# facebookresearch/atlas

Hardware: NVIDIA B200
Metric: end-to-end queries/sec (retrieve top-40 + FiD-base fwd) (higher is better)
Workload: dtype bf16

## Files before the change

### atlas_b200/csrc/gemm.cu

```cuda
#include "common.cuh"
#include "host_common.h"

#include <math.h>
#include <stdlib.h>

namespace gemm {

constexpr int BLOCK_M = 128;
constexpr int BLOCK_K = 64;
constexpr int UMMA_K = 16;
constexpr int THREADS = 384;
constexpr int EPI_WARPS = 8;

enum Epilogue { EPI_NONE = 0, EPI_BIAS = 1, EPI_GELU = 2, EPI_RESIDUAL = 3, EPI_GATED = 4 };

template <int BLOCK_N, bool kPair>
struct Cfg {
    static constexpr int CTAS = kPair ? 2 : 1;
    static constexpr int A_BYTES = BLOCK_M * BLOCK_K * 2;
    static constexpr int B_ROWS = BLOCK_N / CTAS;
    static constexpr int B_BYTES = B_ROWS * BLOCK_K * 2;
    static constexpr int STAGE_BYTES = A_BYTES + B_BYTES;
    static constexpr int STAGES = (192 * 1024) / STAGE_BYTES;
    static constexpr int EPI_STAGE_BYTES = BLOCK_N == 256 ? EPI_WARPS * 4096 : 0;
    static constexpr int SMEM_BYTES = STAGES * STAGE_BYTES + EPI_STAGE_BYTES + 1024;
    static constexpr int TMEM_COLS = 2 * BLOCK_N;
    static constexpr int UMMA_M = BLOCK_M * CTAS;
};

struct Params {
    int M, N, K;
    int ldc;
    int ldr;
    int epi;
    const uint16_t* bias;
    const uint16_t* residual;
    uint16_t* C;
    const float* row_ss;
    float* out_ss;
    float rs_eps;
    int splits, kb_per_split;
    float* C32;
    int l2_prefetch;
    int tma_store;
    const int32_t* m_dev;
};

template <bool kBF16>
__device__ __forceinline__ float to_f32(uint16_t h) {
    if constexpr (kBF16) return __bfloat162float(__ushort_as_bfloat16(h));
    return __half2float(__ushort_as_half(h));
}
template <bool kBF16>
__device__ __forceinline__ uint32_t pack2(float a, float b) {
    return ab::pack2_rn<kBF16>(a, b);
}

__device__ __forceinline__ float gelu_erf(float x) {
    const float z = fabsf(x) * 0.70710678118654752f;
    float t, e;
    asm("rcp.approx.ftz.f32 %0, %1;" : "=f"(t) : "f"(fmaf(0.3275911f, z, 1.0f)));
    asm("ex2.approx.ftz.f32 %0, %1;" : "=f"(e) : "f"(-1.4426950408889634f * z * z));
    float poly = fmaf(1.061405429f, t, -1.453152027f);
    poly = fmaf(poly, t, 1.421413741f);
    poly = fmaf(poly, t, -0.284496736f);
    poly = fmaf(poly, t, 0.254829592f);
    const float erfc_abs = poly * t * e;
    const float one_plus_erf = x >= 0.f ? 2.0f - erfc_abs : erfc_abs;
    return 0.5f * x * one_plus_erf;
}
__device__ __forceinline__ float gelu_new(float x) {
    const float u2 = x * (1.5957691216057308f + 0.07135481627260025f * x * x);
    float e, r;
    asm("ex2.approx.ftz.f32 %0, %1;" : "=f"(e) : "f"(-1.4426950408889634f * u2));
    asm("rcp.approx.ftz.f32 %0, %1;" : "=f"(r) : "f"(1.0f + e));
    return x * r;
}

__device__ __forceinline__ uint64_t umma_desc_mn_sw128(uint32_t smem_addr, uint32_t lbo_bytes) {
    uint64_t d = 0;
    d |= static_cast<uint64_t>((smem_addr & 0x3FFFFu) >> 4);
    d |= static_cast<uint64_t>(lbo_bytes >> 4) << 16;
    d |= static_cast<uint64_t>(1024 >> 4) << 32;
    d |= static_cast<uint64_t>(1) << 46;
    d |= static_cast<uint64_t>(2) << 61;
    return d;
}

template <bool kBF16, int BLOCK_N, bool kPair, bool kTN, bool kQuad>
__global__ void __launch_bounds__(THREADS, 1)
gemm_kernel(const __grid_constant__ CUtensorMap tmap_a, const __grid_constant__ CUtensorMap tmap_b,
            const __grid_constant__ CUtensorMap tmap_c, const Params p) {
    using C = Cfg<BLOCK_N, kPair>;
    extern __shared__ uint8_t smem_raw[];
    __shared__ __align__(8) uint64_t full_bar[C::STAGES];
    __shared__ __align__(8) uint64_t empty_bar[C::STAGES];
    __shared__ __align__(8) uint64_t tmem_full_bar[2];
    __shared__ __align__(8) uint64_t tmem_empty_bar[2];
    __shared__ uint32_t tmem_base_smem;

    const uint32_t warp = threadIdx.x >> 5;
    const uint32_t lane = threadIdx.x & 31u;
    const uint32_t smem_base = (ab::smem_u32(smem_raw) + 1023u) & ~1023u;
    uint8_t* smem_gen = smem_raw + (smem_base - ab::smem_u32(smem_raw));

    static_assert(!kQuad || (kPair && !kTN), "the 4-CTA cluster builds on the K-major pair kernel");
    constexpr int CLUSTER = kQuad ? 4 : (kPair ? 2 : 1);
    const uint32_t cluster_rank = kPair ? ab::cluster_ctarank() : 0u;
    const uint32_t cta_rank = cluster_rank & 1u;
    const uint32_t pair_id = kQuad ? (cluster_rank >> 1) : 0u;
    const bool leader = cta_rank == 0;
    const int group = static_cast<int>(blockIdx.x) / CLUSTER;
    const int num_groups = static_cast<int>(gridDim.x) / CLUSTER;
    constexpr int PAIR_M = BLOCK_M * C::CTAS;
    constexpr int TILE_M = PAIR_M * (kQuad ? 2 : 1);
    const int m_rows = p.m_dev != nullptr ? min(p.M, max(__ldg(p.m_dev), 0)) : p.M;
    const int num_m = (m_rows + TILE_M - 1) / TILE_M;
    const int num_n = (p.N + BLOCK_N - 1) / BLOCK_N;
    const int num_tiles = num_m * num_n * p.splits;
    const int num_kb = (p.K + BLOCK_K - 1) / BLOCK_K;

    if (warp == 0 && lane == 0) {
        ab::tma_prefetch_desc(&tmap_a);
        ab::tma_prefetch_desc(&tmap_b);
    }
    if (warp == 1 && lane == 0) {
        for (int s = 0; s < C::STAGES; ++s) {
            ab::mbar_init(&full_bar[s], 1);
            ab::mbar_init(&empty_bar[s], kQuad ? 2 : 1);
        }
        for (int b = 0; b < 2; ++b) {
            ab::mbar_init(&tmem_full_bar[b], 1);
            ab::mbar_init(&tmem_empty_bar[b], EPI_WARPS * C::CTAS);
        }
        ab::fence_barrier_init();
    }
    if (warp == 2) ab::tmem_alloc<C::CTAS>(&tmem_base_smem, C::TMEM_COLS);
    ab::tc_fence_before();
    if constexpr (kPair) {
        ab::cluster_sync_all();
    } else {
        __syncthreads();
    }
    ab::tc_fence_after();
    const uint32_t tmem_base = tmem_base_smem;

    if (warp == 0) {
        if (lane == 0) {
            uint32_t stage = 0, phase = 0;
            for (int t = group; t < num_tiles; t += num_groups) {
                const int tile = t / p.splits, split = t % p.splits;
                const int m_blk = tile / num_n, n_blk = tile % num_n;
                const int a_row = m_blk * TILE_M + static_cast<int>(pair_id) * PAIR_M + static_cast<int>(cta_rank) * BLOCK_M;
                const int b_row = n_blk * BLOCK_N + static_cast<int>(cta_rank) * C::B_ROWS;
                const int kb0 = split * p.kb_per_split, kb1 = min(num_kb, kb0 + p.kb_per_split);
                int pf_row = -1;
                if constexpr (!kTN) {
                    const int t2 = t + num_groups;
                    if (p.l2_prefetch && t2 < num_tiles && (t2 / p.splits) % num_n == 0)
                        pf_row = ((t2 / p.splits) / num_n) * TILE_M + static_cast<int>(pair_id) * PAIR_M +
                                 static_cast<int>(cta_rank) * BLOCK_M;
                }
                for (int kb = kb0; kb < kb1; ++kb) {
                    if (pf_row >= 0) ab::tma_prefetch_2d(&tmap_a, kb * BLOCK_K, pf_row);
                    ab::mbar_wait(&empty_bar[stage], phase ^ 1u, 11);
                    uint8_t* st = smem_gen + stage * C::STAGE_BYTES;
                    if constexpr (kTN) {
                        if constexpr (kPair) {
                            if (leader) ab::mbar_arrive_expect_tx(&full_bar[stage], 2 * C::STAGE_BYTES);
                        } else {
                            ab::mbar_arrive_expect_tx(&full_bar[stage], C::STAGE_BYTES);
                        }
#pragma unroll
                        for (int j = 0; j < BLOCK_M / 64; ++j) {
                            if constexpr (kPair)
                                ab::tma_load_2d_2sm(&tmap_a, &full_bar[stage], st + j * 8192, a_row + 64 * j, kb * BLOCK_K,
                                                    ab::kEvictNormal);
                            else
                                ab::tma_load_2d(&tmap_a, &full_bar[stage], st + j * 8192, a_row + 64 * j, kb * BLOCK_K,
                                                ab::kEvictNormal);
                        }
#pragma unroll
                        for (int j = 0; j < C::B_ROWS / 64; ++j) {
                            if constexpr (kPair)
                                ab::tma_load_2d_2sm(&tmap_b, &full_bar[stage], st + C::A_BYTES + j * 8192, b_row + 64 * j,
                                                    kb * BLOCK_K, ab::kEvictNormal);
                            else
                                ab::tma_load_2d(&tmap_b, &full_bar[stage], st + C::A_BYTES + j * 8192, b_row + 64 * j,
                                                kb * BLOCK_K, ab::kEvictNormal);
                        }
                    } else if constexpr (kQuad) {
                        if (leader) ab::mbar_arrive_expect_tx(&full_bar[stage], 2 * C::STAGE_BYTES);
                        ab::tma_load_2d_2sm(&tmap_a, &full_bar[stage], st, kb * BLOCK_K, a_row, ab::kEvictNormal);
                        ab::tma_load_2d_2sm_mc(&tmap_b, &full_bar[stage], st + C::A_BYTES + pair_id * (64 * BLOCK_K * 2),
                                               kb * BLOCK_K, b_row + static_cast<int>(pair_id) * 64,
                                               static_cast<uint16_t>(0x5u << cta_rank), ab::kEvictLast);
                    } else if constexpr (kPair) {
                        if (leader) ab::mbar_arrive_expect_tx(&full_bar[stage], 2 * C::STAGE_BYTES);
                        ab::tma_load_2d_2sm(&tmap_a, &full_bar[stage], st, kb * BLOCK_K, a_row, ab::kEvictNormal);
                        ab::tma_load_2d_2sm(&tmap_b, &full_bar[stage], st + C::A_BYTES, kb * BLOCK_K, b_row,
                                            ab::kEvictLast);
                    } else {
                        ab::mbar_arrive_expect_tx(&full_bar[stage], C::STAGE_BYTES);
                        ab::tma_load_2d(&tmap_a, &full_bar[stage], st, kb * BLOCK_K, a_row, ab::kEvictNormal);
                        ab::tma_load_2d(&tmap_b, &full_bar[stage], st + C::A_BYTES, kb * BLOCK_K, b_row,
                                        ab::kEvictLast);
                    }
                    if (++stage == C::STAGES) {
                        stage = 0;
                        phase ^= 1u;
                    }
                }
            }
        }
    } else if (warp == 1) {
        if (lane == 0 && leader) {
            constexpr uint32_t idesc = ab::umma_idesc_f16(C::UMMA_M, BLOCK_N, kBF16) | (kTN ? ((1u << 15) | (1u << 16)) : 0u);
            uint32_t stage = 0, phase = 0;
            int it = 0;
            for (int t = group; t < num_tiles; t += num_groups, ++it) {
                const uint32_t buf = it & 1;
                ab::mbar_wait(&tmem_empty_bar[buf], ((it >> 1) & 1) ^ 1u, 12);
                ab::tc_fence_after();
                const uint32_t d_tmem = tmem_base + buf * BLOCK_N;
                const int kb0 = (t % p.splits) * p.kb_per_split, kb1 = min(num_kb, kb0 + p.kb_per_split);
                for (int kb = kb0; kb < kb1; ++kb) {
                    ab::mbar_wait(&full_bar[stage], phase, 13);
                    ab::tc_fence_after();
                    if constexpr (kTN) {
                        const uint64_t adesc0 = umma_desc_mn_sw128(smem_base + stage * C::STAGE_BYTES, 8192);
                        const uint64_t bdesc0 = umma_desc_mn_sw128(smem_base + stage * C::STAGE_BYTES + C::A_BYTES, 8192);
#pragma unroll
                        for (int k = 0; k < BLOCK_K / UMMA_K; ++k) {
                            ab::umma_ss<C::CTAS>(d_tmem, adesc0 + ((k * UMMA_K * 128) >> 4),
                                                 bdesc0 + ((k * UMMA_K * 128) >> 4), idesc, ((kb - kb0) | k) != 0 ? 1u : 0u);
                        }
                    } else {
                        const uint64_t adesc0 = ab::umma_desc_k_sw128(smem_base + stage * C::STAGE_BYTES);
                        const uint64_t bdesc0 = ab::umma_desc_k_sw128(smem_base + stage * C::STAGE_BYTES + C::A_BYTES);
#pragma unroll
                        for (int k = 0; k < BLOCK_K / UMMA_K; ++k) {
                            ab::umma_ss<C::CTAS>(d_tmem, adesc0 + ((k * UMMA_K * 2) >> 4),
                                                 bdesc0 + ((k * UMMA_K * 2) >> 4), idesc, ((kb - kb0) | k) != 0 ? 1u : 0u);
                        }
                    }
                    if constexpr (kQuad) {
                        ab::umma_commit_2sm(&empty_bar[stage], 0xF);
                    } else if constexpr (kPair) {
                        ab::umma_commit_2sm(&empty_bar[stage], 0x3);
                    } else {
                        ab::umma_commit(&empty_bar[stage]);
                    }
                    if (++stage == C::STAGES) {
                        stage = 0;
                        phase ^= 1u;
                    }
                }
                if constexpr (kPair) {
                    ab::umma_commit_2sm(&tmem_full_bar[buf], static_cast<uint16_t>(0x3u << (2 * pair_id)));
                } else {
                    ab::umma_commit(&tmem_full_bar[buf]);
                }
            }
        }
    } else if (warp >= 4) {
        const uint32_t lg = warp & 3u;
        const uint32_t half = (warp - 4u) >> 2;
        constexpr int CHUNKS = BLOCK_N / 64;
        int it = 0;
        for (int t = group; t < num_tiles; t += num_groups, ++it) {
            const uint32_t buf = it & 1;
            const int tile = t / p.splits, split = t % p.splits;
            const int m_blk = tile / num_n, n_blk = tile % num_n;
            const int row = m_blk * TILE_M + static_cast<int>(pair_id) * PAIR_M + static_cast<int>(cta_rank) * BLOCK_M +
                            static_cast<int>(lg * 32 + lane);
            const float rscale = (p.row_ss != nullptr && row < p.M)
                                     ? rsqrtf(__ldg(p.row_ss + row) / static_cast<float>(p.K) + p.rs_eps) : 1.0f;
            float ss_out = 0.f;
            if constexpr (BLOCK_N == 256) {
                if (p.tma_store && p.C32 == nullptr) {
                    uint8_t* stg = smem_gen + C::STAGES * C::STAGE_BYTES + (warp - 4u) * 4096u;
                    const uint32_t swz = lane & 7u;
                    const bool gated = p.epi == EPI_GATED;
                    const int n_groups = gated ? 1 : 2;
                    const int row_warp = m_blk * TILE_M + static_cast<int>(pair_id) * PAIR_M + static_cast<int>(cta_rank) * BLOCK_M +
                                         static_cast<int>(lg * 32);
                    const int acc_col_w = static_cast<int>(half) * (BLOCK_N / 2);
                    const int out_col_w = gated ? n_blk * (BLOCK_N / 2) + static_cast<int>(half) * (BLOCK_N / 4)
                                                : n_blk * BLOCK_N + acc_col_w;
                    const bool use_res = p.epi == EPI_RESIDUAL;
                    uint4 rq[8];
                    auto load_res = [&](int g) {
#pragma unroll
                        for (int i = 0; i < 8; ++i) {
                            const int rr = row_warp + static_cast<int>(lane >> 3) + 4 * i;
                            const int cc = out_col_w + g * 64 + static_cast<int>(lane & 7u) * 8;
                            rq[i] = (rr < p.M && cc < p.N)
                                        ? __ldg(reinterpret_cast<const uint4*>(p.residual + static_cast<size_t>(rr) * p.ldr + cc))
                                        : make_uint4(0u, 0u, 0u, 0u);
                        }
                    };
                    if (use_res) load_res(0);
                    ab::mbar_wait(&tmem_full_bar[buf], (it >> 1) & 1, 14);
                    ab::tc_fence_after();
#pragma unroll 1
                    for (int g = 0; g < n_groups; ++g) {
                        if (lane == 0) ab::tma_store_wait_read();
                        __syncwarp();
                        uint4 rown[8];
                        if (use_res) {
#pragma unroll
                            for (int i = 0; i < 8; ++i) {
                                const uint32_t rr = (lane >> 3) + 4u * i;
                                *reinterpret_cast<uint4*>(stg + rr * 128u + (((lane & 7u) ^ (rr & 7u)) << 4)) = rq[i];
                            }
                            __syncwarp();
#pragma unroll
                            for (int k = 0; k < 8; ++k)
                                rown[k] = *reinterpret_cast<const uint4*>(stg + lane * 128u + ((static_cast<uint32_t>(k) ^ swz) << 4));
                            if (g + 1 < n_groups) load_res(g + 1);
                        }
                        const int chunks_in_group = gated ? 4 : 2;
#pragma unroll 1
                        for (int cg = 0; cg < chunks_in_group; ++cg) {
                            const int c = gated ? cg : g * 2 + cg;
                            const int col_local = acc_col_w + c * 32;
                            const int col0 = n_blk * BLOCK_N + col_local;
                            uint32_t r[32];
                            ab::tmem_ld32(tmem_base + ((lg * 32u) << 16) + buf * BLOCK_N + col_local, r);
                            ab::tmem_ld_wait();
                            if (c == CHUNKS - 1) {
                                ab::tc_fence_before();
                                __syncwarp();
                                if (lane == 0) {
                                    if (leader) ab::mbar_arrive(&tmem_empty_bar[buf]);
                                    else ab::mbar_arrive_cluster(&tmem_empty_bar[buf], 2 * pair_id);
                                }
                            }
                            float v[32];
#pragma unroll
                            for (int j = 0; j < 32; ++j) v[j] = __uint_as_float(r[j]) * rscale;
                            if (p.epi != EPI_NONE && !gated && p.bias != nullptr) {
#pragma unroll
                                for (int j8 = 0; j8 < 4; ++j8) {
                                    if (col0 + j8 * 8 < p.N) {
                                        const uint4 b = __ldg(reinterpret_cast<const uint4*>(p.bias + col0 + j8 * 8));
                                        const uint32_t w[4] = {b.x, b.y, b.z, b.w};
#pragma unroll
                                        for (int e = 0; e < 4; ++e) {
                                            v[j8 * 8 + 2 * e] += to_f32<kBF16>(static_cast<uint16_t>(w[e] & 0xFFFFu));
                                            v[j8 * 8 + 2 * e + 1] += to_f32<kBF16>(static_cast<uint16_t>(w[e] >> 16));
                                        }
                                    }
                                }
                            }
                            if (p.epi == EPI_GELU) {
#pragma unroll
                                for (int j = 0; j < 32; ++j) v[j] = gelu_erf(v[j]);
                            } else if (use_res) {
#pragma unroll
                                for (int j8 = 0; j8 < 4; ++j8) {
                                    const uint4 b = cg ? rown[4 + j8] : rown[j8];
                                    const uint32_t w[4] = {b.x, b.y, b.z, b.w};
#pragma unroll
                                    for (int e = 0; e < 4; ++e) {
                                        v[j8 * 8 + 2 * e] += to_f32<kBF16>(static_cast<uint16_t>(w[e] & 0xFFFFu));
                                        v[j8 * 8 + 2 * e + 1] += to_f32<kBF16>(static_cast<uint16_t>(w[e] >> 16));
                                    }
                                }
                            }
                            if (gated) {
                                uint32_t o[8];
#pragma unroll
                                for (int e = 0; e < 8; ++e)
                                    o[e] = pack2<kBF16>(gelu_new(v[4 * e]) * v[4 * e + 1], gelu_new(v[4 * e + 2]) * v[4 * e + 3]);
#pragma unroll
                                for (int k = 0; k < 2; ++k)
                                    *reinterpret_cast<uint4*>(stg + lane * 128u + ((static_cast<uint32_t>(cg * 2 + k) ^ swz) << 4)) =
                                        make_uint4(o[4 * k], o[4 * k + 1], o[4 * k + 2], o[4 * k + 3]);
                            } else {
#pragma unroll
                                for (int j8 = 0; j8 < 4; ++j8) {
                                    const uint4 o = make_uint4(
                                        pack2<kBF16>(v[j8 * 8 + 0], v[j8 * 8 + 1]), pack2<kBF16>(v[j8 * 8 + 2], v[j8 * 8 + 3]),
                                        pack2<kBF16>(v[j8 * 8 + 4], v[j8 * 8 + 5]), pack2<kBF16>(v[j8 * 8 + 6], v[j8 * 8 + 7]));
                                    *reinterpret_cast<uint4*>(stg + lane * 128u + ((static_cast<uint32_t>(cg * 4 + j8) ^ swz) << 4)) = o;
                                    if (p.out_ss != nullptr && col0 + j8 * 8 < p.N) {
                                        const uint32_t w[4] = {o.x, o.y, o.z, o.w};
#pragma unroll
                                        for (int e = 0; e < 4; ++e) {
                                            const float a = to_f32<kBF16>(static_cast<uint16_t>(w[e] & 0xFFFFu));
                                            const float b = to_f32<kBF16>(static_cast<uint16_t>(w[e] >> 16));
                                            ss_out = fmaf(a, a, fmaf(b, b, ss_out));
                                        }
                                    }
                                }
                            }
                        }
                        ab::fence_proxy_async_smem();
                        __syncwarp();
                        if (lane == 0 && row_warp < p.M) {
                            ab::tma_store_2d(&tmap_c, stg, out_col_w + g * 64, row_warp);
                            ab::tma_store_commit();
                        }
                    }
                    if (p.out_ss != nullptr && row < p.M) atomicAdd(p.out_ss + row, ss_out);
                    continue;
                }
            }
            ab::mbar_wait(&tmem_full_bar[buf], (it >> 1) & 1, 14);
            ab::tc_fence_after();
#pragma unroll 1
            for (int c = 0; c < CHUNKS; ++c) {
                const int col_local = static_cast<int>(half) * (BLOCK_N / 2) + c * 32;
                const int col0 = n_blk * BLOCK_N + col_local;
                uint32_t r[32];
                ab::tmem_ld32(tmem_base + ((lg * 32u) << 16) + buf * BLOCK_N + col_local, r);
                ab::tmem_ld_wait();
                if (c == CHUNKS - 1) {
                    ab::tc_fence_before();
                    __syncwarp();
                    if (lane == 0) {
                        if (leader) ab::mbar_arrive(&tmem_empty_bar[buf]);
                        else ab::mbar_arrive_cluster(&tmem_empty_bar[buf], 2 * pair_id);
                    }
                }
                if (row >= p.M || col0 >= p.N) continue;
                if (p.C32 != nullptr) {
                    float* crow = p.C32 + (static_cast<size_t>(split) * p.M + row) * p.N + col0;
#pragma unroll
                    for (int j4 = 0; j4 < 8; ++j4)
                        if (col0 + j4 * 4 < p.N)
                            *reinterpret_cast<uint4*>(crow + j4 * 4) = make_uint4(r[4 * j4], r[4 * j4 + 1], r[4 * j4 + 2], r[4 * j4 + 3]);
                    continue;
                }
                float v[32];
#pragma unroll
                for (int j = 0; j < 32; ++j) v[j] = __uint_as_float(r[j]) * rscale;
                if (p.epi != EPI_NONE && p.epi != EPI_GATED && p.bias != nullptr) {
#pragma unroll
                    for (int j8 = 0; j8 < 4; ++j8) {
                        if (col0 + j8 * 8 < p.N) {
                            const uint4 b = __ldg(reinterpret_cast<const uint4*>(p.bias + col0 + j8 * 8));
                            const uint32_t w[4] = {b.x, b.y, b.z, b.w};
#pragma unroll
                            for (int e = 0; e < 4; ++e) {
                                v[j8 * 8 + 2 * e] += to_f32<kBF16>(static_cast<uint16_t>(w[e] & 0xFFFFu));
                                v[j8 * 8 + 2 * e + 1] += to_f32<kBF16>(static_cast<uint16_t>(w[e] >> 16));
                            }
                        }
                    }
                }
                if (p.epi == EPI_GELU) {
#pragma unroll
                    for (int j = 0; j < 32; ++j) v[j] = gelu_erf(v[j]);
                } else if (p.epi == EPI_RESIDUAL) {
                    const uint16_t* rrow = p.residual + static_cast<size_t>(row) * p.ldr + col0;
#pragma unroll
                    for (int j8 = 0; j8 < 4; ++j8) {
                        if (col0 + j8 * 8 < p.N) {
                            const uint4 b = __ldg(reinterpret_cast<const uint4*>(rrow + j8 * 8));
                            const uint32_t w[4] = {b.x, b.y, b.z, b.w};
#pragma unroll
                            for (int e = 0; e < 4; ++e) {
                                v[j8 * 8 + 2 * e] += to_f32<kBF16>(static_cast<uint16_t>(w[e] & 0xFFFFu));
                                v[j8 * 8 + 2 * e + 1] += to_f32<kBF16>(static_cast<uint16_t>(w[e] >> 16));
                            }
                        }
                    }
                }
                if (p.epi == EPI_GATED) {
                    uint16_t* crow = p.C + static_cast<size_t>(row) * p.ldc + (col0 >> 1);
                    uint32_t o[8];
#pragma unroll
                    for (int e = 0; e < 8; ++e)
                        o[e] = pack2<kBF16>(gelu_new(v[4 * e]) * v[4 * e + 1], gelu_new(v[4 * e + 2]) * v[4 * e + 3]);
#pragma unroll
                    for (int j8 = 0; j8 < 2; ++j8)
                        if (col0 + j8 * 16 < p.N)
                            *reinterpret_cast<uint4*>(crow + j8 * 8) =
                                make_uint4(o[4 * j8], o[4 * j8 + 1], o[4 * j8 + 2], o[4 * j8 + 3]);
                } else {
                    uint16_t* crow = p.C + static_cast<size_t>(row) * p.ldc + col0;
#pragma unroll
                    for (int j8 = 0; j8 < 4; ++j8) {
                        if (col0 + j8 * 8 < p.N) {
                            const uint4 o = make_uint4(
                                pack2<kBF16>(v[j8 * 8 + 0], v[j8 * 8 + 1]), pack2<kBF16>(v[j8 * 8 + 2], v[j8 * 8 + 3]),
                                pack2<kBF16>(v[j8 * 8 + 4], v[j8 * 8 + 5]), pack2<kBF16>(v[j8 * 8 + 6], v[j8 * 8 + 7]));
                            *reinterpret_cast<uint4*>(crow + j8 * 8) = o;
                            if (p.out_ss != nullptr) {
                                const uint32_t w[4] = {o.x, o.y, o.z, o.w};
#pragma unroll
                                for (int e = 0; e < 4; ++e) {
                                    const float a = to_f32<kBF16>(static_cast<uint16_t>(w[e] & 0xFFFFu));
                                    const float b = to_f32<kBF16>(static_cast<uint16_t>(w[e] >> 16));
                                    ss_out = fmaf(a, a, fmaf(b, b, ss_out));
                                }
                            }
                        }
                    }
                }
            }
            if (p.out_ss != nullptr && row < p.M) atomicAdd(p.out_ss + row, ss_out);
        }
        if constexpr (BLOCK_N == 256) {
            if (lane == 0) ab::tma_store_wait_all();
        }
    }

    ab::tc_fence_before();
    if constexpr (kPair) {
        ab::cluster_sync_all();
    } else {
        __syncthreads();
    }
    if (warp == 2) {
        ab::tc_fence_after();
        ab::tmem_dealloc<C::CTAS>(tmem_base, C::TMEM_COLS);
    }
}

template <bool kBF16>
static int quad_clusters() {
    static int cached = -1;
    if (cached >= 0) return cached;
    using C = Cfg<256, true>;
    auto kernel = gemm_kernel<kBF16, 256, true, false, true>;
    cached = 0;
    if (cudaFuncSetAttribute(kernel, cudaFuncAttributeMaxDynamicSharedMemorySize, C::SMEM_BYTES) != cudaSuccess) return cached;
    cudaLaunchConfig_t cfg = {};
    cfg.gridDim = dim3(static_cast<unsigned>(abh::num_sms() / 4 * 4));
    cfg.blockDim = dim3(THREADS);
    cfg.dynamicSmemBytes = C::SMEM_BYTES;
    cudaLaunchAttribute attr[1];
    attr[0].id = cudaLaunchAttributeClusterDimension;
    attr[0].val.clusterDim.x = 4;
    attr[0].val.clusterDim.y = 1;
    attr[0].val.clusterDim.z = 1;
    cfg.attrs = attr;
    cfg.numAttrs = 1;
    int n = 0;
    if (cudaOccupancyMaxActiveClusters(&n, kernel, &cfg) == cudaSuccess && n > 0) cached = n;
    else (void)cudaGetLastError();
    return cached;
}

template <bool kBF16, int BLOCK_N, bool kPair, bool kTN = false, bool kQuad = false>
static int launch(const CUtensorMap& ta, const CUtensorMap& tb, const Params& p_in, cudaStream_t s) {
    using C = Cfg<BLOCK_N, kPair>;
    Params p = p_in;
    CUtensorMap tc = ta;
    static const bool stage_off = getenv("ATLAS_B200_GEMM_TMA_STORE") != nullptr && getenv("ATLAS_B200_GEMM_TMA_STORE")[0] == '0';
    p.tma_store = 0;
    if (BLOCK_N == 256 && p.C32 == nullptr && !stage_off) {
        const int n_out = p.epi == EPI_GATED ? p.N / 2 : p.N;
        const int rc = abh::make_tmap_2d_16bit(&tc, p.C, static_cast<uint64_t>(p.M), static_cast<uint64_t>(n_out),
                                               static_cast<uint64_t>(p.ldc), 32, 64, kBF16);
        if (rc) return rc;
        p.tma_store = 1;
    }
    static bool attr_set = false;
    if (!attr_set) {
        AB_CUDA_CHECK(cudaFuncSetAttribute(gemm_kernel<kBF16, BLOCK_N, kPair, kTN, kQuad>,
                                           cudaFuncAttributeMaxDynamicSharedMemorySize, C::SMEM_BYTES));
        attr_set = true;
    }
    constexpr int CLUSTER = kQuad ? 4 : C::CTAS;
    const int tile_m = BLOCK_M * CLUSTER;
    const int tiles = ((p.M + tile_m - 1) / tile_m) * ((p.N + BLOCK_N - 1) / BLOCK_N) * p.splits;
    int groups_max = abh::num_sms() / CLUSTER;
    if constexpr (kQuad) groups_max = quad_clusters<kBF16>();
    const int grid = (tiles < groups_max ? tiles : groups_max) * CLUSTER;
    abh::prof_begin(s, abh::PROF_LINEAR);
    if constexpr (kPair) {
        cudaLaunchConfig_t cfg = {};
        cfg.gridDim = dim3(static_cast<unsigned>(grid));
        cfg.blockDim = dim3(THREADS);
        cfg.dynamicSmemBytes = C::SMEM_BYTES;
        cfg.stream = s;
        cudaLaunchAttribute attr[1];
        attr[0].id = cudaLaunchAttributeClusterDimension;
        attr[0].val.clusterDim.x = CLUSTER;
        attr[0].val.clusterDim.y = 1;
        attr[0].val.clusterDim.z = 1;
        cfg.attrs = attr;
        cfg.numAttrs = 1;
        AB_CUDA_CHECK(cudaLaunchKernelEx(&cfg, gemm_kernel<kBF16, BLOCK_N, kPair, kTN, kQuad>, ta, tb, tc, p));
    } else {
        gemm_kernel<kBF16, BLOCK_N, kPair, kTN, kQuad><<<grid, THREADS, C::SMEM_BYTES, s>>>(ta, tb, tc, p);
    }
    if (p.m_dev != nullptr) abh::prof_end_dyn(s, abh::PROF_LINEAR, 2.0 * static_cast<double>(p.N) * p.K, p.m_dev, p.M);
    else abh::prof_end(s, abh::PROF_LINEAR, 2.0 * p.M * static_cast<double>(p.N) * p.K);
    abh::count_launch();
    AB_CUDA_CHECK(cudaGetLastError());
    return ATLAS_B200_OK;
}

template <bool kBF16>
__global__ void __launch_bounds__(256)
splitk_reduce_kernel(const float* __restrict__ part, uint16_t* __restrict__ out, int64_t ldc, int M, int N, int splits) {
    const int64_t vecs = static_cast<int64_t>(M) * (N / 8);
    for (int64_t idx = blockIdx.x * 256ll + threadIdx.x; idx < vecs; idx += gridDim.x * 256ll) {
        const int64_t row = idx / (N / 8);
        const int col = static_cast<int>(idx % (N / 8)) * 8;
        float a[8] = {0.f, 0.f, 0.f, 0.f, 0.f, 0.f, 0.f, 0.f};
        for (int sidx = 0; sidx < splits; ++sidx) {
            const float4* src = reinterpret_cast<const float4*>(part + (static_cast<size_t>(sidx) * M + row) * N + col);
            const float4 x = __ldg(src), y = __ldg(src + 1);
            a[0] += x.x; a[1] += x.y; a[2] += x.z; a[3] += x.w;
            a[4] += y.x; a[5] += y.y; a[6] += y.z; a[7] += y.w;
        }
        *reinterpret_cast<uint4*>(out + row * ldc + col) =
            make_uint4(pack2<kBF16>(a[0], a[1]), pack2<kBF16>(a[2], a[3]), pack2<kBF16>(a[4], a[5]), pack2<kBF16>(a[6], a[7]));
    }
}

}

static thread_local const int32_t* g_next_m_dev = nullptr;

extern "C" {

int atlas_b200_linear_ex(const void* A, int64_t lda, const void* W, int64_t ldw, const void* bias, const void* residual,
                         int64_t ldr, void* C, int64_t ldc, int32_t M, int32_t N, int32_t K, int32_t epilogue,
                         int32_t is_bf16, const float* row_ss, float* out_ss, float rs_eps, void* stream);

int atlas_b200_linear_dynm(const void* A, int64_t lda, const void* W, int64_t ldw, void* C, int64_t ldc, int32_t M_max, int32_t N,
                           int32_t K, const int32_t* m_dev, int32_t is_bf16, void* stream) {
    AB_REQUIRE(m_dev != nullptr, "linear_dynm: m_dev is required");
    g_next_m_dev = m_dev;
    const int rc = atlas_b200_linear_ex(A, lda, W, ldw, nullptr, nullptr, 0, C, ldc, M_max, N, K, gemm::EPI_NONE, is_bf16, nullptr,
                                        nullptr, 0.f, stream);
    g_next_m_dev = nullptr;
    return rc;
}

int atlas_b200_linear_rows(const void* A, int64_t lda, const void* W, int64_t ldw, const void* bias, const void* residual,
                           int64_t ldr, void* C, int64_t ldc, int32_t M_max, int32_t N, int32_t K, int32_t epilogue,
                           int32_t is_bf16, const float* row_ss, float* out_ss, float rs_eps, const int32_t* m_dev, void* stream) {
    g_next_m_dev = m_dev;
    const int rc = atlas_b200_linear_ex(A, lda, W, ldw, bias, residual, ldr, C, ldc, M_max, N, K, epilogue, is_bf16, row_ss, out_ss,
                                        rs_eps, stream);
    g_next_m_dev = nullptr;
    return rc;
}

int atlas_b200_linear(const void* A, int64_t lda, const void* W, int64_t ldw, const void* bias, const void* residual,
                      int64_t ldr, void* C, int64_t ldc, int32_t M, int32_t N, int32_t K, int32_t epilogue,
                      int32_t is_bf16, void* stream) {
    return atlas_b200_linear_ex(A, lda, W, ldw, bias, residual, ldr, C, ldc, M, N, K, epilogue, is_bf16, nullptr, nullptr,
                                0.f, stream);
}

int atlas_b200_linear_ex(const void* A, int64_t lda, const void* W, int64_t ldw, const void* bias, const void* residual,
                         int64_t ldr, void* C, int64_t ldc, int32_t M, int32_t N, int32_t K, int32_t epilogue,
                         int32_t is_bf16, const float* row_ss, float* out_ss, float rs_eps, void* stream) {
    using namespace gemm;
    AB_REQUIRE(M >= 0 && N > 0 && K > 0, "bad GEMM shape M=%d N=%d K=%d", M, N, K);
    if (M == 0) return ATLAS_B200_OK;
    AB_REQUIRE(N % 8 == 0 && K % 8 == 0 && lda % 8 == 0 && ldw % 8 == 0 && ldc % 8 == 0,
               "N, K and the leading dimensions must be multiples of 8 (16-byte rows)");
    AB_REQUIRE(epilogue >= EPI_NONE && epilogue <= EPI_GATED, "unknown epilogue %d", epilogue);
    AB_REQUIRE(epilogue != EPI_RESIDUAL || (residual != nullptr && ldr % 8 == 0), "EPI_RESIDUAL needs a residual");
    AB_REQUIRE(epilogue != EPI_GATED || N % 32 == 0, "EPI_GATED needs N %% 32 == 0");
    AB_REQUIRE((reinterpret_cast<uintptr_t>(C) & 15u) == 0, "C must be 16-byte aligned");
    AB_REQUIRE(out_ss == nullptr || epilogue != EPI_GATED, "out_ss is not available with the gated epilogue");
    Params p;
    p.splits = 1;
    p.kb_per_split = (K + BLOCK_K - 1) / BLOCK_K;
    p.C32 = nullptr;
    static const int pf_on = (getenv("ATLAS_B200_GEMM_PREFETCH") != nullptr && getenv("ATLAS_B200_GEMM_PREFETCH")[0] == '0') ? 0 : 1;
    p.l2_prefetch = pf_on;
    p.m_dev = g_next_m_dev;
    g_next_m_dev = nullptr;
    p.row_ss = row_ss;
    p.out_ss = out_ss;
    p.rs_eps = rs_eps;
    p.M = M;
    p.N = N;
    p.K = K;
    p.ldc = static_cast<int>(ldc);
    p.ldr = static_cast<int>(ldr);
    p.epi = epilogue;
    p.bias = static_cast<const uint16_t*>(bias);
    p.residual = static_cast<const uint16_t*>(residual);
    p.C = static_cast<uint16_t*>(C);
    const bool wide = N >= 256 && (static_cast<int64_t>((M + 127) / 128) * ((N + 255) / 256) >= abh::num_sms() / 2);
    const bool pair = N >= 256 && M >= 256 &&
                      (static_cast<int64_t>((M + 255) / 256) * ((N + 255) / 256) >= abh::num_sms() / 2);
    static const bool quad_off = getenv("ATLAS_B200_GEMM_QUAD") == nullptr || getenv("ATLAS_B200_GEMM_QUAD")[0] != '1';
    static const bool no_pair = getenv("ATLAS_B200_GEMM_NO_PAIR") != nullptr;
    const int qc = (pair && !quad_off && !no_pair && M >= 512) ? (is_bf16 ? quad_clusters<true>() : quad_clusters<false>()) : 0;
    const bool quad = qc > 0 && (static_cast<int64_t>((M + 511) / 512) * ((N + 255) / 256) >= 2ll * qc);
    const int block_n = (wide || pair) ? 256 : 128;
    const int b_box_rows = quad ? 64 : (pair ? 128 : block_n);
    CUtensorMap ta, tb;
    int rc = abh::make_tmap_2d_16bit(&ta, A, static_cast<uint64_t>(M), static_cast<uint64_t>(K),
                                     static_cast<uint64_t>(lda), BLOCK_M, BLOCK_K, is_bf16 != 0);
    if (rc) return rc;
    rc = abh::make_tmap_2d_16bit(&tb, W, static_cast<uint64_t>(N), static_cast<uint64_t>(K), static_cast<uint64_t>(ldw),
                                 static_cast<uint32_t>(b_box_rows), BLOCK_K, is_bf16 != 0);
    if (rc) return rc;
    cudaStream_t s = static_cast<cudaStream_t>(stream);
    if (quad)
        return is_bf16 ? launch<true, 256, true, false, true>(ta, tb, p, s) : launch<false, 256, true, false, true>(ta, tb, p, s);
    if (pair && !no_pair) return is_bf16 ? launch<true, 256, true>(ta, tb, p, s) : launch<false, 256, true>(ta, tb, p, s);
    if (pair && no_pair) {
        rc = abh::make_tmap_2d_16bit(&tb, W, static_cast<uint64_t>(N), static_cast<uint64_t>(K),
                                     static_cast<uint64_t>(ldw), 256, BLOCK_K, is_bf16 != 0);
        if (rc) return rc;
        return is_bf16 ? launch<true, 256, false>(ta, tb, p, s) : launch<false, 256, false>(ta, tb, p, s);
    }
    if (is_bf16) return wide ? launch<true, 256, false>(ta, tb, p, s) : launch<true, 128, false>(ta, tb, p, s);
    return wide ? launch<false, 256, false>(ta, tb, p, s) : launch<false, 128, false>(ta, tb, p, s);
}

static void wgrad_plan(int32_t tokens, int32_t N, int32_t K, bool* pair, int* block_n, int* splits, int* kb_per_split) {
    using namespace gemm;
    *pair = K >= 256 && N >= 256;
    *block_n = K >= 256 ? 256 : 128;
    const int tile_m = *pair ? 256 : 128;
    const int64_t tiles = static_cast<int64_t>((N + tile_m - 1) / tile_m) * ((K + *block_n - 1) / *block_n);
    const int groups = abh::num_sms() / (*pair ? 2 : 1);
    const int num_kb = (tokens + BLOCK_K - 1) / BLOCK_K;
    int best = 1;
    double best_t = 1e30;
    for (int sp = 1; sp <= 16 && sp * 8 <= num_kb; ++sp) {
        const int64_t waves = (tiles * sp + groups - 1) / groups;
        const double t = static_cast<double>(waves) / sp + 0.02 * sp;
        if (t < best_t - 1e-9) {
            best_t = t;
            best = sp;
        }
    }
    const int per = (num_kb + best - 1) / best;
    *kb_per_split = per > 0 ? per : 1;
    *splits = num_kb > 0 ? (num_kb + *kb_per_split - 1) / *kb_per_split : 1;
}

size_t atlas_b200_linear_wgrad_workspace_bytes(int32_t tokens, int32_t N, int32_t K) {
    bool pair;
    int block_n, splits, per;
    wgrad_plan(tokens, N, K, &pair, &block_n, &splits, &per);
    return splits > 1 ? static_cast<size_t>(splits) * N * K * sizeof(float) : 0;
}

int atlas_b200_linear_wgrad(const void* dY, int64_t lddy, const void* X, int64_t ldx, void* dW, int64_t lddw, int32_t tokens,
                            int32_t N, int32_t K, int32_t is_bf16, void* workspace, size_t workspace_bytes, void* stream) {
    using namespace gemm;
    AB_REQUIRE(tokens >= 0 && N > 0 && K > 0, "bad wgrad shape tokens=%d N=%d K=%d", tokens, N, K);
    AB_REQUIRE(N % 8 == 0 && K % 8 == 0 && lddy % 8 == 0 && ldx % 8 == 0 && lddw % 8 == 0,
               "wgrad: N, K and the leading dimensions must be multiples of 8 (16-byte rows)");
    AB_REQUIRE((reinterpret_cast<uintptr_t>(dW) & 15u) == 0, "dW must be 16-byte aligned");
    cudaStream_t s = static_cast<cudaStream_t>(stream);
    if (tokens == 0) {
        AB_CUDA_CHECK(cudaMemset2DAsync(dW, static_cast<size_t>(lddw) * 2, 0, static_cast<size_t>(K) * 2, N, s));
        return ATLAS_B200_OK;
    }
    Params p;
    p.l2_prefetch = 0;
    p.m_dev = nullptr;
    p.row_ss = nullptr;
    p.out_ss = nullptr;
    p.rs_eps = 0.f;
    p.M = N;
    p.N = K;
    p.K = tokens;
    p.ldc = static_cast<int>(lddw);
    p.ldr = 0;
    p.epi = EPI_NONE;
    p.bias = nullptr;
    p.residual = nullptr;
    p.C = static_cast<uint16_t*>(dW);
    bool pair;
    int block_n, splits, per;
    wgrad_plan(tokens, N, K, &pair, &block_n, &splits, &per);
    const bool wide = block_n == 256;
    static const bool no_splitk = getenv("ATLAS_B200_WGRAD_NO_SPLITK") != nullptr;
    const size_t need = static_cast<size_t>(splits) * N * K * sizeof(float);
    if (splits > 1 && (no_splitk || workspace == nullptr || workspace_bytes < need ||
                       (reinterpret_cast<uintptr_t>(workspace) & 15u) != 0)) {
        splits = 1;
        per = (tokens + BLOCK_K - 1) / BLOCK_K;
    }
    p.splits = splits;
    p.kb_per_split = per;
    p.C32 = splits > 1 ? static_cast<float*>(workspace) : nullptr;
    CUtensorMap ta, tb;
    int rc = abh::make_tmap_2d_16bit(&ta, dY, static_cast<uint64_t>(tokens), static_cast<uint64_t>(N),
                                     static_cast<uint64_t>(lddy), BLOCK_K, 64, is_bf16 != 0);
    if (rc) return rc;
    rc = abh::make_tmap_2d_16bit(&tb, X, static_cast<uint64_t>(tokens), static_cast<uint64_t>(K), static_cast<uint64_t>(ldx),
                                 BLOCK_K, 64, is_bf16 != 0);
    if (rc) return rc;
    if (pair) rc = is_bf16 ? launch<true, 256, true, true>(ta, tb, p, s) : launch<false, 256, true, true>(ta, tb, p, s);
    else if (is_bf16) rc = wide ? launch<true, 256, false, true>(ta, tb, p, s) : launch<true, 128, false, true>(ta, tb, p, s);
    else rc = wide ? launch<false, 256, false, true>(ta, tb, p, s) : launch<false, 128, false, true>(ta, tb, p, s);
    if (rc || splits == 1) return rc;
    const int64_t vecs = static_cast<int64_t>(N) * (K / 8);
    const int64_t blocks = (vecs + 255) / 256, cap = static_cast<int64_t>(abh::num_sms()) * 8;
    const int grid = static_cast<int>(blocks < cap ? blocks : cap);
    if (is_bf16) splitk_reduce_kernel<true><<<grid, 256, 0, s>>>(p.C32, p.C, p.ldc, N, K, splits);
    else splitk_reduce_kernel<false><<<grid, 256, 0, s>>>(p.C32, p.C, p.ldc, N, K, splits);
    abh::count_launch();
    AB_CUDA_CHECK(cudaGetLastError());
    return ATLAS_B200_OK;
}

}
```

Measured before the change: 389.2.

## Add split-K with in-kernel serial reduction for small-M forward GEMMs

For forward GEMMs with M≤512 that would fill under half the SMs, a planner now picks BLOCK_N (64 or 128) and a split-K factor. Each split writes fp32 partials to a per-stream workspace, and the last-arriving CTA per tile, tracked by an atomic counter, reduces them and applies the usual epilogue. This targets poor SM occupancy on small decoder and query-side GEMMs, at the cost of extra global traffic for partials and a new BLOCK_N=64 instantiation. The epilogue is factored into a shared lambda.

```diff
diff --git a/atlas_b200/csrc/gemm.cu b/atlas_b200/csrc/gemm.cu
--- a/atlas_b200/csrc/gemm.cu
+++ b/atlas_b200/csrc/gemm.cu
@@ -3,6 +3,10 @@
 
 #include <math.h>
 #include <stdlib.h>
+
+#include <map>
+#include <mutex>
+#include <utility>
 
 namespace gemm {
 
@@ -41,6 +45,8 @@
     float rs_eps;
     int splits, kb_per_split;
     float* C32;
+    float* ws;
+    int* tile_cnt;
     int l2_prefetch;
     int tma_store;
     const int32_t* m_dev;
@@ -98,6 +104,7 @@
     __shared__ __align__(8) uint64_t tmem_full_bar[2];
     __shared__ __align__(8) uint64_t tmem_empty_bar[2];
     __shared__ uint32_t tmem_base_smem;
+    __shared__ int last_smem;
 
     const uint32_t warp = threadIdx.x >> 5;
     const uint32_t lane = threadIdx.x & 31u;
@@ -408,8 +415,135 @@
                     continue;
                 }
             }
+            auto finish = [&](float (&v)[32], int col0) {
+                if (p.epi != EPI_NONE && p.epi != EPI_GATED && p.bias != nullptr) {
+#pragma unroll
+                    for (int j8 = 0; j8 < 4; ++j8) {
+                        if (col0 + j8 * 8 < p.N) {
+                            const uint4 b = __ldg(reinterpret_cast<const uint4*>(p.bias + col0 + j8 * 8));
+                            const uint32_t w[4] = {b.x, b.y, b.z, b.w};
+#pragma unroll
+                            for (int e = 0; e < 4; ++e) {
+                                v[j8 * 8 + 2 * e] += to_f32<kBF16>(static_cast<uint16_t>(w[e] & 0xFFFFu));
+                                v[j8 * 8 + 2 * e + 1] += to_f32<kBF16>(static_cast<uint16_t>(w[e] >> 16));
+                            }
+                        }
+                    }
+                }
+                if (p.epi == EPI_GELU) {
+#pragma unroll
+                    for (int j = 0; j < 32; ++j) v[j] = gelu_erf(v[j]);
+                } else if (p.epi == EPI_RESIDUAL) {
+                    const uint16_t* rrow = p.residual + static_cast<size_t>(row) * p.ldr + col0;
+#pragma unroll
+                    for (int j8 = 0; j8 < 4; ++j8) {
+                        if (col0 + j8 * 8 < p.N) {
+                            const uint4 b = __ldg(reinterpret_cast<const uint4*>(rrow + j8 * 8));
+                            const uint32_t w[4] = {b.x, b.y, b.z, b.w};
+#pragma unroll
+                            for (int e = 0; e < 4; ++e) {
+                                v[j8 * 8 + 2 * e] += to_f32<kBF16>(static_cast<uint16_t>(w[e] & 0xFFFFu));
+                                v[j8 * 8 + 2 * e + 1] += to_f32<kBF16>(static_cast<uint16_t>(w[e] >> 16));
+                            }
+                        }
+                    }
+                }
+                if (p.epi == EPI_GATED) {
+                    uint16_t* crow = p.C + static_cast<size_t>(row) * p.ldc + (col0 >> 1);
+                    uint32_t o[8];
+#pragma unroll
+                    for (int e = 0; e < 8; ++e)
+                        o[e] = pack2<kBF16>(gelu_new(v[4 * e]) * v[4 * e + 1], gelu_new(v[4 * e + 2]) * v[4 * e + 3]);
+#pragma unroll
+                    for (int j8 = 0; j8 < 2; ++j8)
+                        if (col0 + j8 * 16 < p.N)
+                            *reinterpret_cast<uint4*>(crow + j8 * 8) =
+                                make_uint4(o[4 * j8], o[4 * j8 + 1], o[4 * j8 + 2], o[4 * j8 + 3]);
+                } else {
+                    uint16_t* crow = p.C + static_cast<size_t>(row) * p.ldc + col0;
+#pragma unroll
+                    for (int j8 = 0; j8 < 4; ++j8) {
+                        if (col0 + j8 * 8 < p.N) {
+                            const uint4 o = make_uint4(
+                                pack2<kBF16>(v[j8 * 8 + 0], v[j8 * 8 + 1]), pack2<kBF16>(v[j8 * 8 + 2], v[j8 * 8 + 3]),
+                                pack2<kBF16>(v[j8 * 8 + 4], v[j8 * 8 + 5]), pack2<kBF16>(v[j8 * 8 + 6], v[j8 * 8 + 7]));
+                            *reinterpret_cast<uint4*>(crow + j8 * 8) = o;
+                            if (p.out_ss != nullptr) {
+                                const uint32_t w[4] = {o.x, o.y, o.z, o.w};
+#pragma unroll
+                                for (int e = 0; e < 4; ++e) {
+                                    const float a = to_f32<kBF16>(static_cast<uint16_t>(w[e] & 0xFFFFu));
+                                    const float b = to_f32<kBF16>(static_cast<uint16_t>(w[e] >> 16));
+                                    ss_out = fmaf(a, a, fmaf(b, b, ss_out));
+                                }
+                            }
+                        }
+                    }
+                }
+            };
             ab::mbar_wait(&tmem_full_bar[buf], (it >> 1) & 1, 14);
             ab::tc_fence_after();
+            if (!kPair && !kTN && p.ws != nullptr) {
+                constexpr int SLOT_F4 = BLOCK_M * BLOCK_N / 4;
+                const uint32_t rl = lg * 32u + lane;
+                float4* part = reinterpret_cast<float4*>(p.ws) + static_cast<size_t>(t) * SLOT_F4;
+#pragma unroll 1
+                for (int c = 0; c < CHUNKS; ++c) {
+                    const int cg = static_cast<int>(half) * CHUNKS + c;
+                    uint32_t r[32];
+                    ab::tmem_ld32(tmem_base + ((lg * 32u) << 16) + buf * BLOCK_N + cg * 32, r);
+                    ab::tmem_ld_wait();
+                    if (c == CHUNKS - 1) {
+                        ab::tc_fence_before();
+                        __syncwarp();
+                        if (lane == 0) ab::mbar_arrive(&tmem_empty_bar[buf]);
+                    }
+#pragma unroll
+                    for (int j4 = 0; j4 < 8; ++j4)
+                        __stcg(part + (cg * 8 + j4) * BLOCK_M + rl,
+                               make_float4(__uint_as_float(r[4 * j4]), __uint_as_float(r[4 * j4 + 1]),
+                                           __uint_as_float(r[4 * j4 + 2]), __uint_as_float(r[4 * j4 + 3])));
+                }
+                __threadfence();
+                asm volatile("bar.sync 1, %0;" ::"n"(EPI_WARPS * 32) : "memory");
+                if (threadIdx.x == 4 * 32) {
+                    const int arrived = atomicAdd(p.tile_cnt + tile, 1) + 1;
+                    last_smem = arrived == p.splits ? 1 : 0;
+                    if (arrived == p.splits) p.tile_cnt[tile] = 0;
+                }
+                asm volatile("bar.sync 1, %0;" ::"n"(EPI_WARPS * 32) : "memory");
+                if (!last_smem) continue;
+                __threadfence();
+                if (row >= p.M) continue;
+                const float4* tile_part = reinterpret_cast<const float4*>(p.ws) + static_cast<size_t>(tile) * p.splits * SLOT_F4;
+#pragma unroll 1
+                for (int c = 0; c < CHUNKS; ++c) {
+                    const int cg = static_cast<int>(half) * CHUNKS + c;
+                    const int col0 = n_blk * BLOCK_N + cg * 32;
+                    if (col0 >= p.N) continue;
+                    float v[32];
+#pragma unroll
+                    for (int j = 0; j < 32; ++j) v[j] = 0.f;
+#pragma unroll 1
+                    for (int sp = 0; sp < p.splits; ++sp) {
+                        float4 x[8];
+#pragma unroll
+                        for (int j4 = 0; j4 < 8; ++j4) x[j4] = __ldcg(tile_part + static_cast<size_t>(sp) * SLOT_F4 + (cg * 8 + j4) * BLOCK_M + rl);
+#pragma unroll
+                        for (int j4 = 0; j4 < 8; ++j4) {
+                            v[4 * j4] += x[j4].x;
+                            v[4 * j4 + 1] += x[j4].y;
+                            v[4 * j4 + 2] += x[j4].z;
+                            v[4 * j4 + 3] += x[j4].w;
+                        }
+                    }
+#pragma unroll
+                    for (int j = 0; j < 32; ++j) v[j] *= rscale;
+                    finish(v, col0);
+                }
+                if (p.out_ss != nullptr) atomicAdd(p.out_ss + row, ss_out);
+                continue;
+            }
 #pragma unroll 1
             for (int c = 0; c < CHUNKS; ++c) {
                 const int col_local = static_cast<int>(half) * (BLOCK_N / 2) + c * 32;
@@ -437,70 +571,7 @@
                 float v[32];
 #pragma unroll
                 for (int j = 0; j < 32; ++j) v[j] = __uint_as_float(r[j]) * rscale;
-                if (p.epi != EPI_NONE && p.epi != EPI_GATED && p.bias != nullptr) {
-#pragma unroll
-                    for (int j8 = 0; j8 < 4; ++j8) {
-                        if (col0 + j8 * 8 < p.N) {
-                            const uint4 b = __ldg(reinterpret_cast<const uint4*>(p.bias + col0 + j8 * 8));
-                            const uint32_t w[4] = {b.x, b.y, b.z, b.w};
-#pragma unroll
-                            for (int e = 0; e < 4; ++e) {
-                                v[j8 * 8 + 2 * e] += to_f32<kBF16>(static_cast<uint16_t>(w[e] & 0xFFFFu));
-                                v[j8 * 8 + 2 * e + 1] += to_f32<kBF16>(static_cast<uint16_t>(w[e] >> 16));
-                            }
-                        }
-                    }
-                }
-                if (p.epi == EPI_GELU) {
-#pragma unroll
-                    for (int j = 0; j < 32; ++j) v[j] = gelu_erf(v[j]);
-                } else if (p.epi == EPI_RESIDUAL) {
-                    const uint16_t* rrow = p.residual + static_cast<size_t>(row) * p.ldr + col0;
-#pragma unroll
-                    for (int j8 = 0; j8 < 4; ++j8) {
-                        if (col0 + j8 * 8 < p.N) {
-                            const uint4 b = __ldg(reinterpret_cast<const uint4*>(rrow + j8 * 8));
-                            const uint32_t w[4] = {b.x, b.y, b.z, b.w};
-#pragma unroll
-                            for (int e = 0; e < 4; ++e) {
-                                v[j8 * 8 + 2 * e] += to_f32<kBF16>(static_cast<uint16_t>(w[e] & 0xFFFFu));
-                                v[j8 * 8 + 2 * e + 1] += to_f32<kBF16>(static_cast<uint16_t>(w[e] >> 16));
-                            }
-                        }
-                    }
-                }
-                if (p.epi == EPI_GATED) {
-                    uint16_t* crow = p.C + static_cast<size_t>(row) * p.ldc + (col0 >> 1);
-                    uint32_t o[8];
-#pragma unroll
-                    for (int e = 0; e < 8; ++e)
-                        o[e] = pack2<kBF16>(gelu_new(v[4 * e]) * v[4 * e + 1], gelu_new(v[4 * e + 2]) * v[4 * e + 3]);
-#pragma unroll
-                    for (int j8 = 0; j8 < 2; ++j8)
-                        if (col0 + j8 * 16 < p.N)
-                            *reinterpret_cast<uint4*>(crow + j8 * 8) =
-                                make_uint4(o[4 * j8], o[4 * j8 + 1], o[4 * j8 + 2], o[4 * j8 + 3]);
-                } else {
-                    uint16_t* crow = p.C + static_cast<size_t>(row) * p.ldc + col0;
-#pragma unroll
-                    for (int j8 = 0; j8 < 4; ++j8) {
-                        if (col0 + j8 * 8 < p.N) {
-                            const uint4 o = make_uint4(
-                                pack2<kBF16>(v[j8 * 8 + 0], v[j8 * 8 + 1]), pack2<kBF16>(v[j8 * 8 + 2], v[j8 * 8 + 3]),
-                                pack2<kBF16>(v[j8 * 8 + 4], v[j8 * 8 + 5]), pack2<kBF16>(v[j8 * 8 + 6], v[j8 * 8 + 7]));
-                            *reinterpret_cast<uint4*>(crow + j8 * 8) = o;
-                            if (p.out_ss != nullptr) {
-                                const uint32_t w[4] = {o.x, o.y, o.z, o.w};
-#pragma unroll
-                                for (int e = 0; e < 4; ++e) {
-                                    const float a = to_f32<kBF16>(static_cast<uint16_t>(w[e] & 0xFFFFu));
-                                    const float b = to_f32<kBF16>(static_cast<uint16_t>(w[e] >> 16));
-                                    ss_out = fmaf(a, a, fmaf(b, b, ss_out));
-                                }
-                            }
-                        }
-                    }
-                }
+                finish(v, col0);
             }
             if (p.out_ss != nullptr && row < p.M) atomicAdd(p.out_ss + row, ss_out);
         }
@@ -618,6 +689,61 @@
 
 }
 
+static void smallm_plan(int M, int N, int K, int* block_n, int* splits, int* kb_per_split) {
+    using namespace gemm;
+    const int num_kb = (K + BLOCK_K - 1) / BLOCK_K;
+    const int m_blocks = (M + BLOCK_M - 1) / BLOCK_M;
+    double best = 1e30;
+    *block_n = 128;
+    *splits = 1;
+    *kb_per_split = num_kb;
+    for (int bn = 64; bn <= 128; bn *= 2) {
+        const int tiles = m_blocks * ((N + bn - 1) / bn);
+        for (int sp = 1; sp <= 16; ++sp) {
+            const int per = (num_kb + sp - 1) / sp;
+            const int used = (num_kb + per - 1) / per;
+            if (used != sp || (sp > 1 && per < 2) || static_cast<int64_t>(tiles) * sp > abh::num_sms()) continue;
+            const double tile_bytes = static_cast<double>(BLOCK_M) * bn * 4;
+            const double cost = per * static_cast<double>((BLOCK_M + bn) * BLOCK_K * 2) + (sp > 1 ? 0.5 * (sp + 1) * tile_bytes : 0.0);
+            if (cost < best - 1e-9) {
+                best = cost;
+                *block_n = bn;
+                *splits = sp;
+                *kb_per_split = per;
+            }
+        }
+    }
+}
+
+static int splitk_workspace(cudaStream_t stream, float** ws, int** cnt) {
+    struct Region {
+        float* ws;
+        int* cnt;
+    };
+    static std::mutex mu;
+    static std::map<std::pair<int, cudaStream_t>, Region> regions;
+    int dev = 0;
+    AB_CUDA_CHECK(cudaGetDevice(&dev));
+    std::lock_guard<std::mutex> lock(mu);
+    auto it = regions.find({dev, stream});
+    if (it == regions.end()) {
+        const size_t ws_bytes = static_cast<size_t>(abh::num_sms()) * gemm::BLOCK_M * 128 * sizeof(float);
+        const size_t cnt_bytes = static_cast<size_t>(abh::num_sms()) * sizeof(int);
+        void* mem = nullptr;
+        cudaStreamCaptureMode mode = cudaStreamCaptureModeRelaxed;
+        AB_CUDA_CHECK(cudaThreadExchangeStreamCaptureMode(&mode));
+        const cudaError_t e = cudaMalloc(&mem, ws_bytes + cnt_bytes);
+        AB_CUDA_CHECK(cudaThreadExchangeStreamCaptureMode(&mode));
+        AB_CUDA_CHECK(e);
+        Region r{static_cast<float*>(mem), reinterpret_cast<int*>(static_cast<char*>(mem) + ws_bytes)};
+        AB_CUDA_CHECK(cudaMemsetAsync(r.cnt, 0, cnt_bytes, stream));
+        it = regions.emplace(std::make_pair(dev, stream), r).first;
+    }
+    *ws = it->second.ws;
+    *cnt = it->second.cnt;
+    return ATLAS_B200_OK;
+}
+
 static thread_local const int32_t* g_next_m_dev = nullptr;
 
 extern "C" {
@@ -670,6 +796,8 @@
     p.splits = 1;
     p.kb_per_split = (K + BLOCK_K - 1) / BLOCK_K;
     p.C32 = nullptr;
+    p.ws = nullptr;
+    p.tile_cnt = nullptr;
     static const int pf_on = (getenv("ATLAS_B200_GEMM_PREFETCH") != nullptr && getenv("ATLAS_B200_GEMM_PREFETCH")[0] == '0') ? 0 : 1;
     p.l2_prefetch = pf_on;
     p.m_dev = g_next_m_dev;
@@ -693,7 +821,20 @@
     static const bool no_pair = getenv("ATLAS_B200_GEMM_NO_PAIR") != nullptr;
     const int qc = (pair && !quad_off && !no_pair && M >= 512) ? (is_bf16 ? quad_clusters<true>() : quad_clusters<false>()) : 0;
     const bool quad = qc > 0 && (static_cast<int64_t>((M + 511) / 512) * ((N + 255) / 256) >= 2ll * qc);
-    const int block_n = (wide || pair) ? 256 : 128;
+    const char* smallm_env = getenv("ATLAS_B200_GEMM_SMALLM");
+    const bool smallm = p.m_dev == nullptr && M <= 512 && !(smallm_env != nullptr && smallm_env[0] == '0') &&
+                        static_cast<int64_t>((M + 127) / 128) * ((N + 127) / 128) < abh::num_sms() / 2;
+    int block_n = (wide || pair) ? 256 : 128;
+    if (smallm) {
+        int splits, per;
+        smallm_plan(M, N, K, &block_n, &splits, &per);
+        if (splits > 1) {
+            const int rc = splitk_workspace(static_cast<cudaStream_t>(stream), &p.ws, &p.tile_cnt);
+            if (rc) return rc;
+            p.splits = splits;
+            p.kb_per_split = per;
+        }
+    }
     const int b_box_rows = quad ? 64 : (pair ? 128 : block_n);
     CUtensorMap ta, tb;
     int rc = abh::make_tmap_2d_16bit(&ta, A, static_cast<uint64_t>(M), static_cast<uint64_t>(K),
@@ -703,6 +844,10 @@
                                  static_cast<uint32_t>(b_box_rows), BLOCK_K, is_bf16 != 0);
     if (rc) return rc;
     cudaStream_t s = static_cast<cudaStream_t>(stream);
+    if (smallm) {
+        if (block_n == 64) return is_bf16 ? launch<true, 64, false>(ta, tb, p, s) : launch<false, 64, false>(ta, tb, p, s);
+        return is_bf16 ? launch<true, 128, false>(ta, tb, p, s) : launch<false, 128, false>(ta, tb, p, s);
+    }
     if (quad)
         return is_bf16 ? launch<true, 256, true, false, true>(ta, tb, p, s) : launch<false, 256, true, false, true>(ta, tb, p, s);
     if (pair && !no_pair) return is_bf16 ? launch<true, 256, true>(ta, tb, p, s) : launch<false, 256, true>(ta, tb, p, s);
@@ -759,6 +904,8 @@
         return ATLAS_B200_OK;
     }
     Params p;
+    p.ws = nullptr;
+    p.tile_cnt = nullptr;
     p.l2_prefetch = 0;
     p.m_dev = nullptr;
     p.row_ss = nullptr;
```

New measurement: 396.1, median of 6. Within noise of the previous version (+1.8%).
